# pweigmann/harmonic-power-flow

Measured on AMD Instinct MI355X. Metric: NR iterations/sec + ms/iter, 1 000-bus x 25-harmonic feeder; |dV| vs reference, higher is better.
Workload: dtype f64

## Files before the change

harmonic-power-flow_amd/csrc/hpf_quad.hpp:

```cpp
#pragma once

template <int CTRL>
__device__ __forceinline__ double dpp_f64(double v) {
    int lo = __double2loint(v), hi = __double2hiint(v);
    lo = __builtin_amdgcn_update_dpp(lo, lo, CTRL, 0xf, 0xf, false);
    hi = __builtin_amdgcn_update_dpp(hi, hi, CTRL, 0xf, 0xf, false);
    return __hiloint2double(hi, lo);
}

__device__ __forceinline__ double row_sum16(double v) {
    v += dpp_f64<0xB1>(v);
    v += dpp_f64<0x4E>(v);
    v += dpp_f64<0x141>(v);
    v += dpp_f64<0x140>(v);
    return v;
}

__device__ __forceinline__ Blk2 blk_current(cplx y, cplx Uj, cplx Ej) {
    Blk2 b;
    b.dV = cmul_unf(y, Ej);
    b.dA = cmul_unf(cmulj(y), Uj);
    return b;
}
__device__ __forceinline__ Blk2 blk_current_diag(cplx y, cplx U, cplx E, cplx yn, bool nonlinear) {
    Blk2 b = blk_current(y, U, E);
    if (nonlinear) {
        b.dV = csub(b.dV, cmul_unf(yn, E));
        b.dA = csub(b.dA, cmul_unf(cmulj(yn), U));
    }
    return b;
}
__device__ __forceinline__ Blk2 blk_power_off(cplx y, cplx Ui, cplx Uj, cplx Ej) {
    const cplx yu = cmul_unf(y, Uj);
    const cplx ye = cmul_unf(y, Ej);
    Blk2 b;
    b.dV = cmul_unf(Ui, cconj(ye));
    b.dA = cmul_unf(cmulj(Ui), cconj(cneg(yu)));
    return b;
}
__device__ __forceinline__ Blk2 blk_power_diag(cplx y, cplx U, cplx E, cplx I) {
    const cplx yu = cmul_unf(y, U);
    const cplx ye = cmul_unf(y, E);
    Blk2 b;
    b.dV = cadd(cmul_unf(E, cconj(I)), cmul_unf(U, cconj(ye)));
    b.dA = cmul_unf(cmulj(U), cconj(csub(I, yu)));
    return b;
}
__device__ __forceinline__ void mask_block(int n, int c, int q, int i, int j, const Blk2& blk, double out[4]) {
#pragma unroll
    for (int tr = 0; tr < 2; ++tr)
#pragma unroll
        for (int tc = 0; tc < 2; ++tc)
            out[tr * 2 + tc] = (loc_valid(n, c, i, 2 * q + tr) && loc_valid(n, c, j, 2 * q + tc)) ? pick(blk, tr, tc) : 0.0;
}

template <int B>
struct TileIO {
    static constexpr int NT = (B + 16) / 16;
    static constexpr int LW = (B + 1 - 16 * (NT - 1)) <= 8 ? 8 : 16;
    static constexpr int RG = (NT - 1) * 64 + 4 * LW;
    static constexpr int NE = B / 4, NP = NE / 2;
    static_assert(NE == 2 * NP + 1, "odd number of row groups");
    __device__ static __forceinline__ size_t off2(int p, int wv, int lg, int jj) {
        return (size_t)p * 2 * RG + (wv < NT - 1 ? wv * 128 + (lg * 16 + jj) * 2 : (NT - 1) * 128 + (lg * LW + jj) * 2);
    }
    __device__ static __forceinline__ size_t off1(int wv, int lg, int jj) {
        return (size_t)NP * 2 * RG + (wv < NT - 1 ? wv * 64 + lg * 16 + jj : (NT - 1) * 64 + lg * LW + jj);
    }
    __device__ static __forceinline__ size_t off(int tr, int reg, int wv, int lg, int jj) {
        const int e = tr * 4 + reg;
        return e < 2 * NP ? off2(e >> 1, wv, lg, jj) + (e & 1) : off1(wv, lg, jj);
    }
    __device__ static __forceinline__ bool ok(int wv, int jj) { return wv < NT - 1 || jj < LW; }
    __device__ static __forceinline__ void load(const double* base, int wv, int lg, int jj, double (&v)[NT * 4]) {
        const bool in = ok(wv, jj);
#pragma unroll
        for (int p = 0; p < NP; ++p) {
            double2 t = {0.0, 0.0};
            if (in) t = *reinterpret_cast<const double2*>(base + off2(p, wv, lg, jj));
            v[2 * p] = t.x;
            v[2 * p + 1] = t.y;
        }
        v[NE - 1] = in ? base[off1(wv, lg, jj)] : 0.0;
    }
    __device__ static __forceinline__ void store(double* base, int wv, int lg, int jj, const double (&v)[NT * 4]) {
        if (!ok(wv, jj)) return;
#pragma unroll
        for (int p = 0; p < NP; ++p) *reinterpret_cast<double2*>(base + off2(p, wv, lg, jj)) = double2{v[2 * p], v[2 * p + 1]};
        base[off1(wv, lg, jj)] = v[NE - 1];
    }
};

template <int NT>
__device__ __forceinline__ void lz_aop(const double* p, double (&a)[NT]) {
    if constexpr (NT % 2 == 0) {
#pragma unroll
        for (int t2 = 0; t2 < NT / 2; ++t2) {
            const double2 v = *reinterpret_cast<const double2*>(p + 2 * t2);
            a[2 * t2] = v.x;
            a[2 * t2 + 1] = v.y;
        }
    } else {
#pragma unroll
        for (int t = 0; t < NT; ++t) a[t] = p[t];
    }
}

#define HPF_WAVE_LDS_FENCE() asm volatile("s_waitcnt lgkmcnt(0)" ::: "memory")

#ifndef HPF_LEAF_XCD
#define HPF_LEAF_XCD 1
#endif
#ifndef HPF_Q100L_OCC
#define HPF_Q100L_OCC 2
#endif
#ifndef HPF_Q100_OCC
#define HPF_Q100_OCC 2
#endif
#ifndef HPF_Q_OCC
#define HPF_Q_OCC 4
#endif

template <int B>
struct FqLds {
    static constexpr int NT = (B + 16) / 16, RP = 16 * NT > 64 ? 16 * NT : 64;
    cplx* ynl;
    double* tab;
    double* dgb;
    double (*cc)[RP * 3];
    double (*panel)[NT * 64];
    double (*wl)[16];
    double (*pv)[16];
    double* gl;
    double* hl;
    double* slb;
    double* gl2;
    double* hl2;
    double* pbuf;
    __device__ __forceinline__ static FqLds carve(double* smem_) {
        FqLds L;
        L.ynl = reinterpret_cast<cplx*>(smem_);
        L.tab = smem_ + 2 * (B / 2) * (B / 2);
        L.dgb = L.tab + (B / 2) * 8;
        L.cc = reinterpret_cast<double (*)[RP * 3]>(L.dgb + RP * 3);
        L.panel = reinterpret_cast<double (*)[NT * 64]>(L.dgb + RP * 3 + NT * RP * 3);
        L.wl = reinterpret_cast<double (*)[16]>(L.dgb + RP * 3 + NT * RP * 3 + 2 * NT * 64);
        L.pv = reinterpret_cast<double (*)[16]>(L.dgb + RP * 3 + NT * RP * 3 + 2 * NT * 64 + 32);
        L.gl = L.dgb + RP * 3 + NT * RP * 3 + 2 * NT * 64 + 64;
        L.hl = L.gl + NT * 32;
        L.slb = L.hl + NT * 32;
        L.gl2 = B <= 52 ? L.slb : L.slb + 2;
        L.hl2 = L.gl2 + NT * 32;
        L.pbuf = smem_;
        return L;
    }
};

template <int B>
constexpr int factor_q_lds() {
    constexpr int NT = (B + 16) / 16, RP = 16 * NT > 64 ? 16 * NT : 64;
    return (B / 2) * 8 + RP * 3 + NT * RP * 3 + 2 * NT * 64 + 32 + 32 + NT * 32 + NT * 32 + 2 * (B / 2) * (B / 2) +
           (B <= 52 ? 2 * B * 10 + 200 + 4 : 2 + 2 * NT * 32);
}
static_assert(factor_q_lds<52>() >= 52 * 53 && factor_q_lds<28>() >= 28 * 29 && factor_q_lds<12>() >= 12 * 13 && factor_q_lds<100>() >= 64 * 101,
              "dense-push buffer of a compress step fits the factor body's LDS");

template <int B, bool LEAF>
__device__ __forceinline__ void factor_q_body(
    const FqLds<B>& lds_, const int bx_, const int by_, const Model& M, const TreeDev& T, const int* __restrict__ nodes, int b, int N, int Nc, const int* __restrict__ active,
    const cplx* __restrict__ Uall, const cplx* __restrict__ Eall, const double* __restrict__ fall, double* __restrict__ Zall,
    double* __restrict__ wall, const double* __restrict__ linAall, double* __restrict__ Call, double* __restrict__ Hall,
    const cplx* __restrict__ I0all, const double* __restrict__ chG, const double* __restrict__ chH,
    const double* __restrict__ chD, const double* __restrict__ chy, const double* __restrict__ Minv,
    double* __restrict__ lfK, double* __restrict__ lfS, long long* __restrict__ dbg, int ablate, int s0,
    int* __restrict__ pivflag, double piv_limit, unsigned long long* __restrict__ tstamp) {
    constexpr int NT = (B + 16) / 16;
    constexpr size_t CT = (size_t)NT * NT * 256;
    constexpr int tcB = B >> 4, jjB = B & 15;
    constexpr int RP = 16 * NT > 64 ? 16 * NT : 64;
    constexpr bool SPECIAL = B <= 52;
    HPF_STAMP_DECL;
#ifdef HPF_FACTOR_STAMPS
    long long sa = 0, sc = 0, gown = 0, gwait = 0, gmf = 0;
#endif
    HPF_STAMP(st0);
    const int s = active ? active[by_ + s0] : (int)by_ + s0;
    if (s < 0) return;
    if (tstamp && threadIdx.x == 0) atomicMin(tstamp, (unsigned long long)wall_clock64());
    const int4* nd = reinterpret_cast<const int4*>(nodes) + (FDESC / 4) * (size_t)bx_;
    const int4 nd0 = nd[0], nd1 = nd[1], nd2 = nd[2], nd3 = nd[3];
    const int k = nd0.x, par = nd0.y, diag_e = nd0.z, devk = nd0.w;
    const int e_dn_k = nd1.x, e_up_k = nd1.y, lin_beg = nd1.z, lin_end = nd1.z + nd1.w;
    const int den_beg = nd2.x, n_den = nd2.y;
    const bool via_chain = (nd3.z & 1) != 0;
    const bool lazy_leaf = SPECIAL && (nd3.z & 2) != 0;
    const int cleafv = nd3.w;
    const bool cleaf = LEAF || cleafv > 0;
    const bool sleaf = SPECIAL && !LEAF && (nd3.z & 4) != 0;
    const bool slback = SPECIAL && !LEAF && (nd3.z & 8) != 0;
    const bool lazy = SPECIAL && !LEAF && cleafv < 0;
    const bool cleafr = cleaf || sleaf;
    int4 cpA = {0, 0, 0, 0}, cpB = {0, 0, 0, 0};
    if (!LEAF) {
        cpA = nd[10];
        cpB = nd[11];
    }
    const int crole = LEAF ? 0 : cpA.x;
    const bool cmp_v = crole == 1, cmp_c = crole == 2;
    const int cmp_ci = cpA.y;
    int4 lzA = {0, 0, -1, -1}, lzB = {-1, -1, 0, 0}, lzC = {-1, -1, 0, 0};
    if (lazy) {
        lzA = nd[7];
        lzB = nd[8];
        lzC = nd[9];
    }
#ifdef HPF_FACTOR_STAMPS
    long long sd1 = 0, sd2 = 0, sd3 = 0, se1 = 0, se2 = 0;
    {
        int kk = k;
        asm volatile("" : "+s"(kk));
        sd1 = __builtin_amdgcn_s_memtime();
    }
#endif
    const int tid = threadIdx.x, lane = tid & 63, lg = lane >> 4, jj = lane & 15;
    const int wv = __builtin_amdgcn_readfirstlane(tid >> 6);
    const int n = M.n, c = M.c, Hn = M.Hn;
    const size_t so = (size_t)s * n * Hn;
    const cplx* U = Uall + so;
    const cplx* E = Eall + so;
    const double* Cs = Call + (size_t)s * n * CT;

    cplx* const ynl = lds_.ynl;
    double* const tab = lds_.tab;
    double* const dgb = lds_.dgb;
    double (*const cc)[RP * 3] = lds_.cc;
    double (*const panel)[NT * 64] = lds_.panel;
    double (*const wl)[16] = lds_.wl;
    double (*const pv)[16] = lds_.pv;
    double* const gl = lds_.gl;
    double* const hl = lds_.hl;
    double* const slb = lds_.slb;

    const bool nl = k >= M.m && M.coupled;
    const int col = 16 * wv + jj, p = col >> 1, t1 = col & 1;
    const int t = lg & 1;

    if (nl && !cleafr && wv >= NT / 2) {
        constexpr int YT = 64 * (NT - NT / 2);
        constexpr int YNL = ((B / 2) * (B / 2) + YT - 1) / YT;
        const double2* ynd = reinterpret_cast<const double2*>(M.YN + (size_t)devk * Hn * Hn);
        double2* yl = reinterpret_cast<double2*>(ynl);
        const int t0 = tid - 64 * (NT / 2);
        if constexpr (YNL <= 6) {
            double2 y0 = {0.0, 0.0}, y1 = y0, y2 = y0, y3 = y0, y4 = y0, y5 = y0;
            if (YNL > 0 && t0 < Hn * Hn) y0 = ynd[t0];
            if (YNL > 1 && t0 + YT < Hn * Hn) y1 = ynd[t0 + YT];
            if (YNL > 2 && t0 + 2 * YT < Hn * Hn) y2 = ynd[t0 + 2 * YT];
            if (YNL > 3 && t0 + 3 * YT < Hn * Hn) y3 = ynd[t0 + 3 * YT];
            if (YNL > 4 && t0 + 4 * YT < Hn * Hn) y4 = ynd[t0 + 4 * YT];
            if (YNL > 5 && t0 + 5 * YT < Hn * Hn) y5 = ynd[t0 + 5 * YT];
            __builtin_amdgcn_sched_barrier(0);
            if (YNL > 0 && t0 < Hn * Hn) yl[t0] = y0;
            if (YNL > 1 && t0 + YT < Hn * Hn) yl[t0 + YT] = y1;
            if (YNL > 2 && t0 + 2 * YT < Hn * Hn) yl[t0 + 2 * YT] = y2;
            if (YNL > 3 && t0 + 3 * YT < Hn * Hn) yl[t0 + 3 * YT] = y3;
            if (YNL > 4 && t0 + 4 * YT < Hn * Hn) yl[t0 + 4 * YT] = y4;
            if (YNL > 5 && t0 + 5 * YT < Hn * Hn) yl[t0 + 5 * YT] = y5;
        } else {
            for (int i = t0; i < Hn * Hn; i += YT) yl[i] = ynd[i];
        }
// ... 499 lines not shown
                if (j < m) {
                    const double cand = used ? -1.0 : fabs(row[j]);
                    double mx = cand;
                    mx = fmax(mx, dpp_f64<0xB1>(mx));
                    mx = fmax(mx, dpp_f64<0x4E>(mx));
                    mx = fmax(mx, dpp_f64<0x141>(mx));
                    mx = fmax(mx, dpp_f64<0x140>(mx));
                    const unsigned long long bal = __builtin_amdgcn_ballot_w64(!used && cand == mx);
                    const int pi = __builtin_ctzll(bal | (1ull << 63));
                    double prow[10];
#pragma unroll
                    for (int c2 = 0; c2 < 10; ++c2)
                        prow[c2] = __hiloint2double(__builtin_amdgcn_readlane(__double2hiint(row[c2]), pi),
                                                    __builtin_amdgcn_readlane(__double2loint(row[c2]), pi));
                    const double ipv = 1.0 / prow[j];
                    const bool me = lane == pi;
                    const double f = me ? 0.0 : row[j] * ipv;
#pragma unroll
                    for (int c2 = 0; c2 < 10; ++c2)
                        row[c2] = c2 == j ? (me ? ipv : -f) : (me ? prow[c2] * ipv : fma(-f, prow[c2], row[c2]));
                    used = used || me;
                    mycol = me ? j : mycol;
                    pcol[j] = pi;
                }
            }
            if (lane < m) {
#pragma unroll
                for (int c2 = 0; c2 < 10; ++c2)
                    if (c2 < m) aug[mycol * 20 + m + pcol[c2]] = row[c2];
            }
            if (slback) {
                double* tk = Zall + ((size_t)s * n + k) * CT;
                if (lane < m) {
#pragma unroll
                    for (int c2 = 0; c2 < 10; ++c2)
                        if (c2 < m) tk[mycol * 10 + pcol[c2]] = row[c2];
                }
                if (lane < 4) tk[100 + lane] = aug[10 * 20 + lane];
            }
        }
        if (slback && tid < Hn * 4) lfS[(so + (size_t)k * Hn) * 4 + tid] = tab[tid];
        __syncthreads();
        {
            double mv[NT * 4];
#pragma unroll
            for (int e = 0; e < NT * 4; ++e) mv[e] = 0.0;
            TileIO<B>::load(Minv + (size_t)(lzB.z - 1) * CT, wv, lg, jj, mv);
#pragma unroll
            for (int e = 0; e < NT * 4; ++e) ct[e >> 2][e & 3] = mv[e];
        }
        {
            double qb[10];
#pragma unroll
            for (int j = 0; j < 10; ++j) qb[j] = (j < m && col < b) ? qbl[j * b + col] : 0.0;
            if (col < 2) {
                const double* wi = aug + 10 * 20;
                qb[0] = wi[col];
                qb[1] = wi[2 + col];
            }
#pragma unroll
            for (int ch = 0; ch < 3; ++ch) {
                if (4 * ch < m) {
                    const int i = 4 * ch + lg;
                    const double* wr = aug + (i < m ? i : 0) * 20 + m;
                    double bop = 0.0;
#pragma unroll
                    for (int j = 0; j < 10; ++j)
                        if (j < m) bop = fma(wr[j], qb[j], bop);
                    bop = i < m ? bop : 0.0;
#pragma unroll
                    for (int tr = 0; tr < NT; ++tr) {
                        const int prow_ = 16 * tr + jj;
                        const double aop = (prow_ < b && i < m) ? pbl[prow_ * m + i] : 0.0;
                        ct[tr] = __builtin_amdgcn_mfma_f64_16x16x4f64(aop, bop, ct[tr], 0, 0, 0);
                    }
                }
            }
        }
        const double yc = col < B ? dgb[col * 3 + 2] : 0.0;
#pragma unroll
        for (int tr = 0; tr < NT; ++tr)
#pragma unroll
            for (int reg = 0; reg < 4; ++reg) {
                if (16 * tr + 4 * reg >= B) continue;
                const int row = 16 * tr + 4 * reg + lg;
                double v = row < b ? ct[tr][reg] : 0.0;
                const double pr = xor16_f64(v);
                const double* si = tab + (row >> 1) * 4 + 2 * t;
                v = t ? fma(si[1], v, si[0] * pr) : fma(si[1], pr, si[0] * v);
                ct[tr][reg] = v;
                const double sm = row_sum16(v * yc);
                if (jj == 0) panel[0][wv * 64 + row] = sm;
            }
        __syncthreads();
        if (wv == tcB && jj == jjB) {
#pragma unroll
            for (int tr = 0; tr < NT; ++tr)
#pragma unroll
                for (int reg = 0; reg < 4; ++reg) {
                    if (16 * tr + 4 * reg >= B) continue;
                    const int row = 16 * tr + 4 * reg + lg;
                    double acc = panel[0][row];
#pragma unroll
                    for (int w2 = 1; w2 < NT; ++w2) acc += panel[0][w2 * 64 + row];
                    ct[tr][reg] = acc;
                }
        }
        HPF_STAMP(st1);
        HPF_STAMP(st3);
    } else {
    if (nl) {
        const int pp = p < B / 2 ? p : 0;
        const double P = tab[t * (B / 2) * 4 + pp * 4 + 2 * t1];
        const double Q = tab[t * (B / 2) * 4 + pp * 4 + 2 * t1 + 1];
        const cplx* yn = ynl + (p < Hn ? p : 0);
#pragma unroll
        for (int tr = 0; tr < NT; ++tr)
#pragma unroll
            for (int reg = 0; reg < 4; ++reg) {
                const int q = 8 * tr + 2 * reg + (lg >> 1);
                const cplx y = yn[(q < Hn ? q : 0) * Hn];
                ct[tr][reg] = y.im * P + y.re * Q;
            }
    }
    HPF_STAMP(sc);
    __syncthreads();
    {
        const bool cvalid = col < b && (col >= 2 || (col == 0 ? k >= 1 : k >= c));
        const bool colB = col == B, colgt = col > B;
        const int dsel = colB ? 2 : t1;
#pragma unroll
        for (int tr = 0; tr < NT; ++tr)
#pragma unroll
            for (int reg = 0; reg < 4; ++reg) {
                const int row = 16 * tr + 4 * reg + lg;
                const double ident = (row == col) ? 1.0 : 0.0;
                if (16 * tr + 4 * reg >= B) {
                    ct[tr][reg] = ident;
                } else {
                    bool rv = row < b;
                    if (tr == 0 && reg == 0) rv = rv && (lg >= 2 || (lg == 0 ? k >= 1 : k >= c));
                    const double dv = dgb[row * 3 + dsel];
                    double v = ct[tr][reg];
                    v = ((row >> 1) == p) ? dv : v;
                    v = (rv && cvalid) ? v : ident;
                    v = colB ? dv : v;
                    v = colgt ? 0.0 : v;
                    ct[tr][reg] = v;
                }
            }
    }
    HPF_STAMP(st1);

    for (int i = 1; i < n_den; ++i) {
        const int ch = i == 1 ? nd2.w : (i == 2 ? nd3.x : (i == 3 ? nd3.y : T.dchild[den_beg + i]));
        const double* Cc = Cs + (size_t)ch * CT;
        double tmp[NT * 4];
        TileIO<B>::load(Cc, wv, lg, jj, tmp);
        __builtin_amdgcn_sched_barrier(0);
#pragma unroll
        for (int e = 0; e < NT * 4; ++e)
            if (16 * (e >> 2) + 4 * (e & 3) < B) sumc[e] += tmp[e];
        __builtin_amdgcn_sched_barrier(0);
    }
    if (cmp_c) {
        double tmp[NT * 4];
        TileIO<B>::load(T.cF + ((size_t)s * T.n_comp + cmp_ci) * 3 * CT, wv, lg, jj, tmp);
        __builtin_amdgcn_sched_barrier(0);
#pragma unroll
        for (int e = 0; e < NT * 4; ++e)
            if (16 * (e >> 2) + 4 * (e & 3) < B) sumc[e] += tmp[e];
    }
#pragma unroll
    for (int e = 0; e < NT * 4; ++e)
        if (16 * (e >> 2) + 4 * (e & 3) < B) ct[e >> 2][e & 3] -= sumc[e];

    HPF_STAMP(st3);
    constexpr int NB16 = B / 16;
    if constexpr (NB16 > 0) {
        constexpr int WS = 17, NBUF = NB16 > 1 ? 2 : 1;
        static_assert(2 * (B / 2) * (B / 2) + (B / 2) * 8 + RP * 3 + NT * RP * 3 >= NBUF * NT * 16 * WS, "block images fit the dead assembly arrays");
        double* const img = lds_.pbuf;
        double* const pcol = &panel[1][0];
        __syncthreads();
#pragma unroll
        for (int T = 0; T < NB16; ++T) {
            double* const im = img + (size_t)(NBUF > 1 ? (T & 1) : 0) * NT * 16 * WS;
#ifdef HPF_FACTOR_STAMPS
            const long long g0_ = __builtin_amdgcn_s_memtime();
#endif
            if (wv == T) {
#pragma unroll
                for (int ss = 0; ss < 4; ++ss) {
                    const int j0 = 4 * ss;
                    const bool incol = jj >= j0 && jj < j0 + 4;
                    if (incol) pv[0][lg * 4 + (jj - j0)] = ct[T][ss];
                    HPF_WAVE_LDS_FENCE();
                    bool weak;
                    const double wji = inv4_cofactor_lane(pv[0], lane, piv_limit, weak);
                    if (incol) {
#pragma unroll
                        for (int reg = 0; reg < 4; ++reg) pcol[(lg + 4 * reg) * 4 + (jj - j0)] = ct[T][reg];
                    }
                    if (weak && lane < 16) atomicOr(pivflag + s, 1);
                    if (lane < 16) wl[0][(lane & 3) * 4 + (lane >> 2)] = wji;
                    HPF_WAVE_LDS_FENCE();
                    const double vcol = pcol[jj * 4 + lg];
                    const double aopl = incol ? 0.0 : vcol;
                    const double aw = jj < 4 ? wl[0][jj * 4 + lg] : 0.0;
                    const d4_t z = {0.0, 0.0, 0.0, 0.0};
                    const d4_t d = __builtin_amdgcn_mfma_f64_16x16x4f64(aw, ct[T][ss], z, 0, 0, 0);
                    double rfin = d[0];
                    if (incol) {
                        rfin = wl[0][lg * 4 + (jj - j0)];
                        ct[T] = d4_t{0.0, 0.0, 0.0, 0.0};
                    }
                    ct[T] = __builtin_amdgcn_mfma_f64_16x16x4f64(aopl, -rfin, ct[T], 0, 0, 0);
                    ct[T][ss] = rfin;
                    HPF_WAVE_LDS_FENCE();
                }
#pragma unroll
                for (int tr = 0; tr < NT; ++tr)
#pragma unroll
                    for (int reg = 0; reg < 4; ++reg) im[tr * 16 * WS + (4 * reg + lg) * WS + jj] = ct[tr][reg];
            }
#ifdef HPF_FACTOR_STAMPS
            const long long g1_ = __builtin_amdgcn_s_memtime();
#endif
            __syncthreads();
#ifdef HPF_FACTOR_STAMPS
            const long long g2_ = __builtin_amdgcn_s_memtime();
#endif
            d4_t Rn;
            if (wv == T) {
                Rn = -ct[T];
            } else {
                d4_t r4 = {0.0, 0.0, 0.0, 0.0};
#pragma unroll
                for (int k4 = 0; k4 < 4; ++k4) r4 = __builtin_amdgcn_mfma_f64_16x16x4f64(im[T * 16 * WS + jj * WS + 4 * k4 + lg], ct[T][k4], r4, 0, 0, 0);
                ct[T] = r4;
                Rn = -r4;
            }
#pragma unroll
            for (int tr = 0; tr < NT; ++tr) {
                if (tr == T) continue;
                d4_t a4 = ct[tr];
                if (wv == T) a4 = d4_t{0.0, 0.0, 0.0, 0.0};
#pragma unroll
                for (int k4 = 0; k4 < 4; ++k4) a4 = __builtin_amdgcn_mfma_f64_16x16x4f64(im[tr * 16 * WS + jj * WS + 4 * k4 + lg], Rn[k4], a4, 0, 0, 0);
                ct[tr] = a4;
            }
#ifdef HPF_FACTOR_STAMPS
            {
                asm volatile("" : "+v"(ct[0]), "+v"(ct[NT - 1]));
                const long long g3_ = __builtin_amdgcn_s_memtime();
                if (T == 0) gown += g1_ - g0_;
                gwait += g2_ - g1_;
                gmf += g3_ - g2_;
            }
#endif
        }
    }
#pragma unroll
    for (int st = 4 * NB16; st < B / 4; ++st) {
        {
            const int tP = st >> 2, rg = st & 3, j0 = 4 * (st & 3), buf = st & 1;
            const bool incol = jj >= j0 && jj < j0 + 4;
#ifdef HPF_FACTOR_STAMPS
            const long long g0_ = __builtin_amdgcn_s_memtime();
#endif
            if (wv == tP) {
                if (incol) pv[buf][lg * 4 + (jj - j0)] = ct[tP][rg];
                bool weak;
                const double wji = inv4_cofactor_lane(pv[buf], lane, piv_limit, weak);
                if (incol) {
#pragma unroll
                    for (int tr = 0; tr < NT; ++tr)
#pragma unroll
                        for (int reg = 0; reg < 4; ++reg) panel[buf][(16 * tr + lg + 4 * reg) * 4 + (jj - j0)] = ct[tr][reg];
                }
                if (weak && lane < 16) atomicOr(pivflag + s, 1);
                if (lane < 16) wl[buf][(lane & 3) * 4 + (lane >> 2)] = wji;
            }
#ifdef HPF_FACTOR_STAMPS
            const long long g1_ = __builtin_amdgcn_s_memtime();
#endif
            __syncthreads();
#ifdef HPF_FACTOR_STAMPS
            const long long g2_ = __builtin_amdgcn_s_memtime();
#endif
            double aop[NT];
#pragma unroll
            for (int tr = 0; tr < NT; ++tr) {
                const double v = panel[buf][(16 * tr + jj) * 4 + lg];
                aop[tr] = (tr == tP && incol) ? 0.0 : -v;
            }
            const double aw = jj < 4 ? wl[buf][jj * 4 + lg] : 0.0;
            const d4_t z = {0.0, 0.0, 0.0, 0.0};
            const d4_t d = __builtin_amdgcn_mfma_f64_16x16x4f64(aw, ct[tP][rg], z, 0, 0, 0);
            double rfin = d[0];
            if (wv == tP && incol) {
                rfin = wl[buf][lg * 4 + (jj - j0)];
#pragma unroll
                for (int tr = 0; tr < NT; ++tr) ct[tr] = d4_t{0.0, 0.0, 0.0, 0.0};
            }
#pragma unroll
            for (int tr = 0; tr < NT; ++tr) ct[tr] = __builtin_amdgcn_mfma_f64_16x16x4f64(aop[tr], rfin, ct[tr], 0, 0, 0);
            ct[tP][rg] = rfin;
#ifdef HPF_FACTOR_STAMPS
            {
                const long long g3_ = __builtin_amdgcn_s_memtime();
                if (tP == 0) gown += g1_ - g0_;
                gwait += g2_ - g1_;
                gmf += g3_ - g2_;
            }
#endif
        }
    }

    }
    HPF_STAMP(st4);
    {
        double* Zk = Zall + ((size_t)s * n + k) * CT;
        if (!cleaf && !slback) {
            double zv[NT * 4];
#pragma unroll
            for (int e = 0; e < NT * 4; ++e) zv[e] = ct[e >> 2][e & 3];
            TileIO<B>::store(Zk, wv, lg, jj, zv);
        }
        if (wv == tcB && jj == jjB) {
            double* wk = wall + ((size_t)s * n + k) * B;
#pragma unroll
            for (int tr = 0; tr < NT; ++tr)
#pragma unroll
                for (int reg = 0; reg < 4; ++reg) {
                    const int row = 16 * tr + lg + 4 * reg;
                    if (row < B) wk[row] = ct[tr][reg];
                }
        }
    }

    HPF_STAMP(st5);
    auto schur_tiles = [&](const double* gsrc, const double* hsrc, const double sign, const bool rhs, double (&cv)[NT * 4]) {
        const int ti = lg & 1, tcn = jj & 1;
        double ha = hsrc[p * 4 + 2 * tcn + tcn];
        double hb = hsrc[p * 4 + 2 * (tcn ^ 1) + tcn];
        if (col == B) {
            ha = rhs ? 1.0 : 0.0;
            hb = 0.0;
        }
        if (col > B) {
            ha = 0.0;
            hb = 0.0;
        }
        ha *= sign;
        hb *= sign;
#pragma unroll
        for (int tr = 0; tr < NT; ++tr)
#pragma unroll
            for (int reg = 0; reg < 4; ++reg) {
                const int q = 8 * tr + 2 * reg + (lg >> 1);
                const double ga = gsrc[q * 4 + 2 * ti + ti];
                const double gb = gsrc[q * 4 + 2 * ti + (ti ^ 1)];
                const double own = ct[tr][reg];
                const double rowp = xor16_f64(own);
                const double colp = xor1_f64(own);
                const double both = xor1_f64(rowp);
                cv[tr * 4 + reg] = fma(gb, fma(both, hb, rowp * ha), ga * fma(colp, hb, own * ha));
            }
    };
    if (B > 52) {
        if (par >= 0 && !cmp_c) {
            double* Ck = Call + ((size_t)s * n + k) * CT;
            const int ti = lg & 1, tcn = jj & 1;
            double ha = hl[p * 4 + 2 * tcn + tcn], hb = hl[p * 4 + 2 * (tcn ^ 1) + tcn];
            if (col == B) {
                ha = 1.0;
                hb = 0.0;
            }
            if (col > B) {
                ha = 0.0;
                hb = 0.0;
            }
            const bool st_ok = TileIO<B>::ok(wv, jj);
            auto one = [&](const int e) {
                const int tr = e >> 2, reg = e & 3;
                const int q = 8 * tr + 2 * reg + (lg >> 1);
                const double ga = gl[q * 4 + 2 * ti + ti], gb = gl[q * 4 + 2 * ti + (ti ^ 1)];
                const double own = ct[tr][reg];
                const double rowp = xor16_f64(own);
                const double colp = xor1_f64(own);
                const double both = xor1_f64(rowp);
                return fma(gb, fma(both, hb, rowp * ha), ga * fma(colp, hb, own * ha));
            };
#pragma unroll
            for (int pp = 0; pp < TileIO<B>::NP; ++pp) {
                const double a = one(2 * pp), b2 = one(2 * pp + 1);
                if (st_ok) *reinterpret_cast<double2*>(Ck + TileIO<B>::off2(pp, wv, lg, jj)) = double2{a, b2};
            }
            const double z = one(TileIO<B>::NE - 1);
            if (st_ok) Ck[TileIO<B>::off1(wv, lg, jj)] = z;
        }
    } else if (par >= 0 && !cmp_c && (!lazy_leaf || wv == tcB)) {
        double* Ck = Call + ((size_t)s * n + k) * CT;
        double cv[NT * 4];
        schur_tiles(gl, hl, 1.0, true, cv);
        if (!lazy_leaf) {
            TileIO<B>::store(Ck, wv, lg, jj, cv);
        } else if (col == B) {
#pragma unroll
            for (int e = 0; e < NT * 4; ++e)
                if (16 * (e >> 2) + 4 * (e & 3) < B) Ck[16 * (e >> 2) + 4 * (e & 3) + lg] = cv[e];
        }
    }
    if (!LEAF && cmp_v) {
        double* Fk = T.cF + ((size_t)s * T.n_comp + cmp_ci) * 3 * CT;
        const int ti = lg & 1, tcn = jj & 1;
        const bool mcol = col < B;
        const double ha = mcol ? hl[p * 4 + 2 * tcn + tcn] : 0.0, hb = mcol ? hl[p * 4 + 2 * (tcn ^ 1) + tcn] : 0.0;
        double ha2 = mcol ? lds_.hl2[p * 4 + 2 * tcn + tcn] : 0.0, hb2 = mcol ? lds_.hl2[p * 4 + 2 * (tcn ^ 1) + tcn] : 0.0;
        if (col == B) ha2 = 1.0;
        const bool st_ok = TileIO<B>::ok(wv, jj);
        double* Ga = Fk + CT + ((size_t)(col >> 2) * NT) * 64 + (col & 3) * 16 + lg;
#pragma unroll
        for (int e = 0; e < TileIO<B>::NE; ++e) {
            const int tr = e >> 2, reg = e & 3;
            const int q = 8 * tr + 2 * reg + (lg >> 1);
            const double ga = gl[q * 4 + 2 * ti + ti], gb = gl[q * 4 + 2 * ti + (ti ^ 1)];
            const double ga2 = lds_.gl2[q * 4 + 2 * ti + ti], gb2 = lds_.gl2[q * 4 + 2 * ti + (ti ^ 1)];
            const double own = ct[tr][reg];
            const double rowp = xor16_f64(own);
            const double colp = xor1_f64(own);
            const double both = xor1_f64(rowp);
            const double uh = fma(colp, hb, own * ha), vh = fma(both, hb, rowp * ha);
            const double uh2 = fma(colp, hb2, own * ha2), vh2 = fma(both, hb2, rowp * ha2);
            const double fcc = fma(gb2, vh2, ga2 * uh2);
            const double hd = -fma(gb2, vh, ga2 * uh);
            const double gd = -fma(gb, vh2, ga * uh2);
            if (st_ok) {
                const size_t o = TileIO<B>::off(tr, reg, wv, lg, jj);
                Fk[o] = fcc;
                Fk[2 * CT + o] = hd;
            }
            if (mcol) Ga[tr * 64 + 4 * reg] = gd;
            __builtin_amdgcn_sched_barrier(0);
        }
        if (mcol) {
#pragma unroll
            for (int e = TileIO<B>::NE; e < NT * 4; ++e) Ga[(e >> 2) * 64 + 4 * (e & 3)] = 0.0;
        }
    }
    if (!LEAF && cmp_c && par >= 0) {
        const double* Fk = T.cF + ((size_t)s * T.n_comp + cmp_ci) * 3 * CT;
        const double* Ga = Fk + CT + lane;
        d4_t pt[NT];
#pragma unroll
        for (int tr = 0; tr < NT; ++tr) pt[tr] = d4_t{0.0, 0.0, 0.0, 0.0};
#pragma unroll
        for (int st = 0; st < B / 4; ++st) {
            double aop[NT];
#pragma unroll
            for (int tr = 0; tr < NT; ++tr) aop[tr] = Ga[((size_t)st * NT + tr) * 64];
#pragma unroll
            for (int tr = 0; tr < NT; ++tr) pt[tr] = __builtin_amdgcn_mfma_f64_16x16x4f64(aop[tr], ct[st >> 2][st & 3], pt[tr], 0, 0, 0);
        }
        double hd[NT * 4];
        TileIO<B>::load(Fk + 2 * CT, wv, lg, jj, hd);
        if (col >= B) {
#pragma unroll
            for (int e = 0; e < NT * 4; ++e) hd[e] = 0.0;
        }
        constexpr int PS = B + 1;
        constexpr int TRP = NT < 4 ? NT : 4;
        double* const pl = lds_.pbuf;
        double cv[NT * 4];
#pragma unroll
        for (int tr0 = 0; tr0 < NT; tr0 += TRP) {
            __syncthreads();
#pragma unroll
            for (int tr = tr0; tr < tr0 + TRP && tr < NT; ++tr)
#pragma unroll
                for (int reg = 0; reg < 4; ++reg)
                    if (16 * tr + 4 * reg < B && col < B) pl[(16 * (tr - tr0) + 4 * reg + lg) * PS + col] = pt[tr][reg];
            __syncthreads();
#pragma unroll
            for (int tr = tr0; tr < tr0 + TRP && tr < NT; ++tr) {
                d4_t acc = {0.0, 0.0, 0.0, 0.0};
                const int prow = 16 * (tr - tr0) + jj;
#pragma unroll
                for (int st = 0; st < B / 4; ++st) {
                    const double a = (16 * tr + jj < B) ? pl[prow * PS + 4 * st + lg] : 0.0;
                    acc = __builtin_amdgcn_mfma_f64_16x16x4f64(a, hd[st], acc, 0, 0, 0);
                }
#pragma unroll
                for (int reg = 0; reg < 4; ++reg) cv[tr * 4 + reg] = col == B ? pt[tr][reg] : acc[reg];
            }
        }
        TileIO<B>::store(Call + ((size_t)s * n + k) * CT, wv, lg, jj, cv);
    }
    if (tstamp) {
        __syncthreads();
        if (threadIdx.x == 0) atomicMax(tstamp + 1, (unsigned long long)wall_clock64());
    }
#ifdef HPF_FACTOR_STAMPS
    if ((ablate & 16) && tid == 0 && dbg) {
        st6 = __builtin_amdgcn_s_memtime();
        long long* o = dbg + ((size_t)s * n + k) * 8;
        o[0] = st1 - st0;
        o[1] = (((sa - st0) >> 4) & 0xffff) | ((((sc - sa) >> 4) & 0xffff) << 16) | (1ll << 62);
        o[4] = (((sd1 - st0) >> 4) & 0xffff) | ((((sd2 - sd1) >> 4) & 0xffff) << 16) | ((((sd3 - sd2) >> 4) & 0xffff) << 32) |
               ((((sa - sd3) >> 4) & 0xffff) << 48);
        o[2] = ((gown >> 4) & 0xfffff) | (((gwait >> 4) & 0xfffff) << 20) | (((gmf >> 4) & 0xfffff) << 40);
        o[3] = st4 - st3;
        o[5] = st6 - st5;
        o[6] = n_den + (sleaf ? 100 : 0);
        o[7] = (k >= M.m) | ((lin_end - lin_beg) << 1) | ((((se1 - sd2) >> 4) & 0xffff) << 16) | ((((se2 ? se2 - se1 : 0) >> 4) & 0xffff) << 32) |
               ((long long)(lzC.x >= 0) << 48) | ((long long)(lzC.y >= 0) << 49) | ((long long)lazy << 50);
    }
#endif
}

template <int B, bool LEAF>
__global__ __launch_bounds__(64 * ((B + 16) / 16), (B > 52 ? (LEAF ? HPF_Q100L_OCC : HPF_Q100_OCC) : (B > 28 ? (LEAF ? 6 : HPF_Q_OCC) : 5))) void k_factor_q(
    Model M, TreeDev T, const int* __restrict__ nodes, int b, int N, int Nc, const int* __restrict__ active,
    const cplx* __restrict__ Uall, const cplx* __restrict__ Eall, const double* __restrict__ fall, double* __restrict__ Zall,
    double* __restrict__ wall, const double* __restrict__ linAall, double* __restrict__ Call, double* __restrict__ Hall,
    const cplx* __restrict__ I0all, const double* __restrict__ chG, const double* __restrict__ chH,
    const double* __restrict__ chD, const double* __restrict__ chy, const double* __restrict__ Minv,
    double* __restrict__ lfK, double* __restrict__ lfS, long long* __restrict__ dbg, int ablate, int s0,
    int* __restrict__ pivflag, double piv_limit, unsigned long long* __restrict__ tstamp, int leaf_count, unsigned leaf_S) {
    constexpr int NT = (B + 16) / 16, RP = 16 * NT > 64 ? 16 * NT : 64;
    FqLds<B> lds;
    if constexpr (LEAF) {
        __shared__ cplx ynl[(B / 2) * (B / 2)];
        __shared__ double tab[(B / 2) * 8], dgb[RP * 3], cc[NT][RP * 3], panel[2][NT * 64], wl[2][16], pv[2][16], gl[NT * 32], hl[NT * 32];
        __shared__ double slb[B <= 52 ? 2 * B * 10 + 200 + 4 : 1];
        lds.ynl = ynl; lds.tab = tab; lds.dgb = dgb; lds.cc = cc; lds.panel = panel; lds.wl = wl; lds.pv = pv; lds.gl = gl; lds.hl = hl; lds.slb = slb;
        lds.gl2 = lds.hl2 = lds.pbuf = nullptr;
    } else {
        __shared__ __attribute__((aligned(16))) double smem[factor_q_lds<B>()];
        lds = FqLds<B>::carve(smem);
    }
    int bx = blockIdx.x, by = blockIdx.y;
#if HPF_LEAF_XCD
    if constexpr (LEAF) {
        const unsigned id = blockIdx.x, t = id >> 3, S_ = gridDim.y == 1 ? leaf_S : 1u;
        by = (int)(t % S_);
        bx = (int)((t / S_) * 8u + (id & 7u));
        if (bx >= leaf_count) return;
    }
#endif
    factor_q_body<B, LEAF>(lds, bx, by, M, T, nodes, b, N, Nc, active, Uall, Eall, fall, Zall, wall, linAall, Call, Hall, I0all, chG,
                           chH, chD, chy, Minv, lfK, lfS, dbg, ablate, s0, pivflag, piv_limit, tstamp);
}

__device__ __forceinline__ void lds_barrier() {
    __builtin_amdgcn_fence(__ATOMIC_RELEASE, "workgroup", "local");
    __builtin_amdgcn_s_barrier();
    __builtin_amdgcn_fence(__ATOMIC_ACQUIRE, "workgroup", "local");
}

template <int B>
struct BackQIn {
    static constexpr int NT = (B + 16) / 16;
    int4 kp;
    int s;
    double x;
    double zr[NT * 4];
    double hk0, hk1, h20, h21;
};

template <int B>
__device__ __forceinline__ void back_q_load(
    BackQIn<B>& in, const int bx_, const int by_, const Model& M, const TreeDev& T, const int* __restrict__ nodes, int b,
    const int* __restrict__ active, const double* __restrict__ Zall, const double* __restrict__ wall, const double* __restrict__ Hall,
    const double* __restrict__ Minv, int s0) {
    constexpr int NT = (B + 16) / 16;
    constexpr size_t CT = (size_t)NT * NT * 256;
    const int s = active ? active[by_ + s0] : (int)by_ + s0;
    in.s = s;
    if (s < 0) return;
    const int4 kp = reinterpret_cast<const int4*>(nodes)[bx_];
    in.kp = kp;
    const int k = kp.x, par = kp.y, cleaf = kp.z;
    const int crole = kp.w >> 28, cinfo = kp.w & 0x0fffffff;
    const int tid = threadIdx.x, lane = tid & 63, lg = lane >> 4, jj = lane & 15;
    const int wv = __builtin_amdgcn_readfirstlane(tid >> 6);
    const int n = M.n, Hn = M.Hn;
    in.x = 0.0;
    if (tid < B) in.x = wall[((size_t)s * n + k) * B + tid];
    if (par >= 0) {
        if (cleaf) {
            TileIO<B>::load(Minv + (size_t)(cleaf - 1) * CT, wv, lg, jj, in.zr);
        } else {
            TileIO<B>::load(Zall + ((size_t)s * n + k) * CT, wv, lg, jj, in.zr);
        }
        const int col = 16 * wv + jj, p = col >> 1, t1 = col & 1;
        if (crole != 2 && col < b) {
            const double* hk = Hall + ((size_t)s * n + k) * Hn * 4 + p * 4 + t1 * 2;
            in.hk0 = hk[0];
            in.hk1 = hk[1];
            if (crole == 1) {
                const double* h2 = T.cH2 + ((size_t)s * T.n_comp + cinfo) * Hn * 4 + p * 4 + t1 * 2;
                in.h20 = h2[0];
                in.h21 = h2[1];
            }
        }
    }
}

template <int B>
__device__ __forceinline__ double back_q_compute(
    const BackQIn<B>& in, const Model& M, const TreeDev& T, int b, int N, int Nc, double* __restrict__ xall, double* __restrict__ step,
    const double* __restrict__ lfK, const double* __restrict__ lfS, const double* xp, const double* xc) {
    constexpr int NT = (B + 16) / 16;
    constexpr size_t CT = (size_t)NT * NT * 256;
    const int s = in.s;
    const int k = in.kp.x, par = in.kp.y, cleaf = in.kp.z;
    const int crole = in.kp.w >> 28, cinfo = in.kp.w & 0x0fffffff;
    const int tid = threadIdx.x, lane = tid & 63, lg = lane >> 4, jj = lane & 15;
    const int wv = __builtin_amdgcn_readfirstlane(tid >> 6);
    const int n = M.n, c = M.c, Hn = M.Hn;
    double* xs = xall + (size_t)s * n * B;
    constexpr int RP = 16 * NT > 64 ? 16 * NT : 64;
    __shared__ double part[NT][RP];
    __shared__ double mcl[RP * 2], zl[RP];
    double x = in.x;
    if (par >= 0) {
        const int col = 16 * wv + jj, p = col >> 1, t1 = col & 1;
        double tv = 0.0;
        if (crole == 2) {
            double hr[NT * 4];
            TileIO<B>::load(T.cF + (((size_t)s * T.n_comp + cinfo) * 3 + 2) * CT, wv, lg, jj, hr);
            const double xpc = col < b ? xp[col] : 0.0;
#pragma unroll
            for (int e = 0; e < NT * 4; ++e)
                if (16 * (e >> 2) + 4 * (e & 3) < B) {
                    const double r = row_sum16(hr[e] * xpc);
                    if (jj == 0) part[wv][16 * (e >> 2) + lg + 4 * (e & 3)] = r;
                }
            lds_barrier();
            if (tid < B) {
                double acc = part[0][tid];
#pragma unroll
                for (int w2 = 1; w2 < NT; ++w2) acc += part[w2][tid];
                zl[tid] = acc;
            }
            lds_barrier();
            tv = col < b ? zl[col] : 0.0;
            lds_barrier();
        } else if (col < b) {
            tv = fma(in.hk1, xp[2 * p + 1], in.hk0 * xp[2 * p]);
            if (crole == 1) tv += fma(in.h21, xc[2 * p + 1], in.h20 * xc[2 * p]);
        }
        if (cleaf && tid < 2) zl[tid] = tv;
        const double tvs = (cleaf && col < 2) ? 0.0 : tv;
        __builtin_amdgcn_sched_barrier(0);
#pragma unroll
        for (int e = 0; e < NT * 4; ++e)
            if (16 * (e >> 2) + 4 * (e & 3) < B) {
                const double r = row_sum16(in.zr[e] * tvs);
                if (jj == 0) part[wv][16 * (e >> 2) + lg + 4 * (e & 3)] = r;
// ... 106 lines not shown
```

Baseline: 159,700.

## Software-pipeline child Schur tile sums and push-GEMM operand loads

The child-contribution summation now double-buffers tile loads in two halves, so the next child's loads are issued while the current one is accumulated. The push GEMM prefetches its A operands several steps ahead in a rotating register buffer and issues the Hd tile loads in two halves partway through the MFMA loop instead of after it. The aim is to hide global-memory latency behind arithmetic, at the cost of higher register pressure, which may reduce occupancy or cause spills. It also adds debug-stamp fields.

Result: no change. 159,300, median of 2 (-0.3%).

```diff
diff --git a/harmonic-power-flow_amd/csrc/hpf_quad.hpp b/harmonic-power-flow_amd/csrc/hpf_quad.hpp
--- a/harmonic-power-flow_amd/csrc/hpf_quad.hpp
+++ b/harmonic-power-flow_amd/csrc/hpf_quad.hpp
@@ -83,6 +83,18 @@
         }
         v[NE - 1] = in ? base[off1(wv, lg, jj)] : 0.0;
     }
+    static_assert(NP >= NT && NE <= 4 * NT, "both halves fit NT * 2 values");
+    template <int HI>
+    __device__ static __forceinline__ void load_half_raw(const double* base, int wv, int lg, int jj, double (&v)[NT * 2]) {
+        const int jc = ok(wv, jj) ? jj : 0;
+#pragma unroll
+        for (int p = HI ? NT : 0; p < (HI ? NP : NT); ++p) {
+            const double2 t = *reinterpret_cast<const double2*>(base + off2(p, wv, lg, jc));
+            v[2 * (p - (HI ? NT : 0))] = t.x;
+            v[2 * (p - (HI ? NT : 0)) + 1] = t.y;
+        }
+        if (HI) v[NE - 1 - 2 * NT] = base[off1(wv, lg, jc)];
+    }
     __device__ static __forceinline__ void store(double* base, int wv, int lg, int jj, const double (&v)[NT * 4]) {
         if (!ok(wv, jj)) return;
 #pragma unroll
@@ -116,6 +128,13 @@
 #endif
 #ifndef HPF_Q100_OCC
 #define HPF_Q100_OCC 2
+#endif
+#ifndef HPF_PUSH_DEPTH
+#define HPF_PUSH_DEPTH 5
+#endif
+#ifndef HPF_PUSH_HD_LO
+#define HPF_PUSH_HD_LO 8
+#define HPF_PUSH_HD_HI 11
 #endif
 #ifndef HPF_Q_OCC
 #define HPF_Q_OCC 4
@@ -921,24 +940,45 @@
     }
     HPF_STAMP(st1);
 
-    for (int i = 1; i < n_den; ++i) {
-        const int ch = i == 1 ? nd2.w : (i == 2 ? nd3.x : (i == 3 ? nd3.y : T.dchild[den_beg + i]));
-        const double* Cc = Cs + (size_t)ch * CT;
-        double tmp[NT * 4];
-        TileIO<B>::load(Cc, wv, lg, jj, tmp);
-        __builtin_amdgcn_sched_barrier(0);
-#pragma unroll
-        for (int e = 0; e < NT * 4; ++e)
-            if (16 * (e >> 2) + 4 * (e & 3) < B) sumc[e] += tmp[e];
-        __builtin_amdgcn_sched_barrier(0);
-    }
-    if (cmp_c) {
-        double tmp[NT * 4];
-        TileIO<B>::load(T.cF + ((size_t)s * T.n_comp + cmp_ci) * 3 * CT, wv, lg, jj, tmp);
-        __builtin_amdgcn_sched_barrier(0);
-#pragma unroll
-        for (int e = 0; e < NT * 4; ++e)
-            if (16 * (e >> 2) + 4 * (e & 3) < B) sumc[e] += tmp[e];
+    {
+        const int n_ch = n_den > 0 ? n_den - 1 : 0, n_mem = n_ch + (cmp_c ? 1 : 0);
+        const double* const cFk = T.cF + ((size_t)s * T.n_comp + cmp_ci) * 3 * CT;
+        int idn = 0;
+        auto member = [&](const int m) -> const double* {
+            if (m >= n_ch) return cFk;
+            const int ch = m == 0 ? nd2.w : (m == 1 ? nd3.x : (m == 2 ? nd3.y : idn));
+            return Cs + (size_t)ch * CT;
+        };
+        if (n_mem > 0) {
+            constexpr int NH = NT * 2, NE = TileIO<B>::NE;
+            double lo[NH], hi[NH];
+            const double* cur = member(0);
+            TileIO<B>::template load_half_raw<0>(cur, wv, lg, jj, lo);
+            TileIO<B>::template load_half_raw<1>(cur, wv, lg, jj, hi);
+            for (int m = 0; m + 1 < n_mem; ++m) {
+                cur = member(m + 1);
+                if (m > 0 && m + 3 < n_den) idn = T.dchild[den_beg + m + 3];
+                __builtin_amdgcn_sched_barrier(0);
+#pragma unroll
+                for (int e = 0; e < NH; ++e) sumc[e] += lo[e];
+                __builtin_amdgcn_sched_barrier(0);
+                TileIO<B>::template load_half_raw<0>(cur, wv, lg, jj, lo);
+                __builtin_amdgcn_sched_barrier(0);
+#pragma unroll
+                for (int e = NH; e < NE; ++e) sumc[e] += hi[e - NH];
+                __builtin_amdgcn_sched_barrier(0);
+                TileIO<B>::template load_half_raw<1>(cur, wv, lg, jj, hi);
+            }
+            __builtin_amdgcn_sched_barrier(0);
+#pragma unroll
+            for (int e = 0; e < NH; ++e) sumc[e] += lo[e];
+#pragma unroll
+            for (int e = NH; e < NE; ++e) sumc[e] += hi[e - NH];
+            if (!TileIO<B>::ok(wv, jj)) {
+#pragma unroll
+                for (int e = 0; e < NE; ++e) sumc[e] = 0.0;
+            }
+        }
     }
 #pragma unroll
     for (int e = 0; e < NT * 4; ++e)
@@ -1225,20 +1265,32 @@
         d4_t pt[NT];
 #pragma unroll
         for (int tr = 0; tr < NT; ++tr) pt[tr] = d4_t{0.0, 0.0, 0.0, 0.0};
+        constexpr int PD = HPF_PUSH_DEPTH < B / 4 ? HPF_PUSH_DEPTH : B / 4;
+        double aop[PD + 1][NT];
+        double hdl[NT * 2], hdh[NT * 2];
+#pragma unroll
+        for (int g = 0; g < PD; ++g)
+#pragma unroll
+            for (int tr = 0; tr < NT; ++tr) aop[g][tr] = Ga[((size_t)g * NT + tr) * 64];
+        constexpr int HLO = (B / 4) * HPF_PUSH_HD_LO / 13, HHI = (B / 4) * HPF_PUSH_HD_HI / 13;
+        static_assert(HLO < B / 4 && HHI < B / 4, "both halves of Hd are requested inside the P loop");
 #pragma unroll
         for (int st = 0; st < B / 4; ++st) {
-            double aop[NT];
-#pragma unroll
-            for (int tr = 0; tr < NT; ++tr) aop[tr] = Ga[((size_t)st * NT + tr) * 64];
-#pragma unroll
-            for (int tr = 0; tr < NT; ++tr) pt[tr] = __builtin_amdgcn_mfma_f64_16x16x4f64(aop[tr], ct[st >> 2][st & 3], pt[tr], 0, 0, 0);
-        }
+            __builtin_amdgcn_sched_barrier(0);
+            if (st == HLO) TileIO<B>::template load_half_raw<0>(Fk + 2 * CT, wv, lg, jj, hdl);
+            if (st == HHI) TileIO<B>::template load_half_raw<1>(Fk + 2 * CT, wv, lg, jj, hdh);
+            if (st + PD < B / 4) {
+#pragma unroll
+                for (int tr = 0; tr < NT; ++tr) aop[(st + PD) % (PD + 1)][tr] = Ga[((size_t)(st + PD) * NT + tr) * 64];
+            }
+            __builtin_amdgcn_sched_barrier(0);
+#pragma unroll
+            for (int tr = 0; tr < NT; ++tr) pt[tr] = __builtin_amdgcn_mfma_f64_16x16x4f64(aop[st % (PD + 1)][tr], ct[st >> 2][st & 3], pt[tr], 0, 0, 0);
+        }
+        HPF_STAMP(st2);
         double hd[NT * 4];
-        TileIO<B>::load(Fk + 2 * CT, wv, lg, jj, hd);
-        if (col >= B) {
-#pragma unroll
-            for (int e = 0; e < NT * 4; ++e) hd[e] = 0.0;
-        }
+#pragma unroll
+        for (int e = 0; e < B / 4; ++e) hd[e] = col >= B ? 0.0 : (e < NT * 2 ? hdl[e] : hdh[e - NT * 2]);
         constexpr int PS = B + 1;
         constexpr int TRP = NT < 4 ? NT : 4;
         double* const pl = lds_.pbuf;
@@ -1276,7 +1328,8 @@
         st6 = __builtin_amdgcn_s_memtime();
         long long* o = dbg + ((size_t)s * n + k) * 8;
         o[0] = st1 - st0;
-        o[1] = (((sa - st0) >> 4) & 0xffff) | ((((sc - sa) >> 4) & 0xffff) << 16) | (1ll << 62);
+        o[1] = (((sa - st0) >> 4) & 0xffff) | ((((sc - sa) >> 4) & 0xffff) << 16) | ((((st3 - st1) >> 4) & 0xffff) << 32) |
+               ((long long)(crole & 3) << 48) | ((((st2 ? st2 - st5 : 0) >> 4) & 0xfff) << 50) | (1ll << 62);
         o[4] = (((sd1 - st0) >> 4) & 0xffff) | ((((sd2 - sd1) >> 4) & 0xffff) << 16) | ((((sd3 - sd2) >> 4) & 0xffff) << 32) |
                ((((sa - sd3) >> 4) & 0xffff) << 48);
         o[2] = ((gown >> 4) & 0xfffff) | (((gwait >> 4) & 0xfffff) << 20) | (((gmf >> 4) & 0xfffff) << 40);
```
